# bramtoula/multi_robot_SLAM_separators

Hardware: AMD Instinct MI355X
Metric: candidate keyframe-pair verifications/sec (NetVLAD NN + ORB match + RANSAC) @1/2/4/8 GPU (higher is better)
Workload: dtype u8+f16+f32+f64

## Files before the change

### include/sepfinder.h

```cpp
#ifndef SEPFINDER_H
#define SEPFINDER_H

#include <stdint.h>
#include <stddef.h>

#ifdef __cplusplus
extern "C" {
#endif

#define SF_ABI_VERSION 8

enum {
  SF_OK = 0,
  SF_EINVAL = 1,
  SF_EHIP = 2,
  SF_ENOMEM = 3,
  SF_ERANGE = 4,
  SF_ENODEV = 5,
  SF_ERCCL = 6
};

#define SF_MAX_FEATURES   32767
#define SF_MAX_DESC_BYTES 64
#define SF_MAX_DESC_BYTES_F32 512
// ... 361 lines not shown
int  sf_prof_get(sf_handle h, int kernel, int64_t* launches, double* total_ms);
const char* sf_kernel_name(int kernel);

enum {
  SF_OPT_MATCH_MFMA = 0,
  SF_OPT_FUSED = 1,
  SF_OPT_OVERLAP = 2,
  SF_OPT_CHAIN_WAVES = 3,
  SF_OPT_NN_FULL_FILTER = 5,
  SF_OPT_STEP_OVERLAP = 6,
  SF_OPT_STEP_SPLIT = 7,
  SF_OPT_STEP_DEPTH = 8,
  SF_OPT_STEP_LANES = 9,
  SF_OPT_STEP_DEVICE_WALK = 10,
  SF_OPT_STEP_SPECULATE = 11,
  SF_OPT_DEBUG_CORR = 4
};
int  sf_set_option(sf_handle h, int32_t option, int32_t value);

#ifdef __cplusplus
}
#endif
#endif
```

### multi_robot_slam_separators_amd/_abi.py

```python
import ctypes as C

import numpy as np

SF_OK, SF_EINVAL, SF_EHIP, SF_ENOMEM, SF_ERANGE, SF_ENODEV, SF_ERCCL = range(7)
SF_MAX_FEATURES = 32767
SF_MAX_DESC_BYTES = 64
SF_MAX_DESC_BYTES_F32 = 512

(SF_K_MATCH, SF_K_RANSAC1, SF_K_GUIDED, SF_K_RANSAC2, SF_K_NN, SF_K_NN_SELECT, SF_K_NN_FILTER,
 SF_K_NN_REFINE, SF_K_FUSED, SF_K_NN_WALK, SF_K_BA, SF_K_GUIDED_TP, SF_K_COUNT) = range(13)
(SF_OPT_MATCH_MFMA, SF_OPT_FUSED, SF_OPT_OVERLAP, SF_OPT_CHAIN_WAVES, SF_OPT_DEBUG_CORR, SF_OPT_NN_FULL_FILTER,
 SF_OPT_STEP_OVERLAP, SF_OPT_STEP_SPLIT, SF_OPT_STEP_DEPTH, SF_OPT_STEP_LANES, SF_OPT_STEP_DEVICE_WALK,
 SF_OPT_STEP_SPECULATE) = range(12)

STATUS_NAMES = {0: "SF_OK", 1: "SF_EINVAL", 2: "SF_EHIP", 3: "SF_ENOMEM", 4: "SF_ERANGE", 5: "SF_ENODEV", 6: "SF_ERCCL"}


class Params(C.Structure):
    _fields_ = [
        ("netvlad_distance", C.c_double),
        ("netvlad_dimensions", C.c_int32),
        ("netvlad_max_matches_nb", C.c_int32),
        ("nn_precision", C.c_int32),
        ("min_inliers", C.c_int32),
        ("inlier_distance", C.c_float),
        ("iterations", C.c_int32),
        ("refine_iterations", C.c_int32),
        ("refine_sigma", C.c_double),
# ... 385 lines not shown
```

### multi_robot_slam_separators_amd/csrc/k_ransac.hip

```cpp
#include "sf_device_math.hpp"
#include "sf_internal.hpp"
#include "k_ba.hip"

namespace {

struct RansacLds {
  float4* src;
  float4* dst;
  float* d2;
  uint8_t* mask_a;
  uint8_t* mask_b;
  double* red;
  unsigned long long* sums;
  int* misc;
  float* hyp;
  int* hyp_cnt;
  float* best;
  float* bc;
  uint32_t* cidx;
};

__device__ __forceinline__ RansacLds ransac_carve(unsigned char* p, int kcap) {
  RansacLds L;
  L.src = (float4*)p; p += (size_t)kcap * 16;
  L.dst = (float4*)p; p += (size_t)kcap * 16;
  L.red = (double*)p; p += 64 * 8;
  L.sums = (unsigned long long*)p; p += 4 * 8;
  L.d2 = (float*)p; p += (size_t)kcap * 4;
  L.misc = (int*)p; p += 16 * 4;
  L.mask_a = p; p += kcap;
  L.mask_b = p; p += kcap;
  L.hyp = (float*)p; p += 12 * 64 * 4;
  L.hyp_cnt = (int*)p; p += 5 * 64 * 4;
  L.best = (float*)p; p += 16 * 4;
  L.bc = (float*)p; p += 16 * 4;
  L.cidx = (uint32_t*)p;
  return L;
}

__device__ __forceinline__ bool draw_sample(const RansacLds& L, uint64_t seed, uint32_t it, int max_checks,
                                            uint32_t m, double sdt, uint32_t& s0, uint32_t& s1, uint32_t& s2) {
  for (int a = 0; a < max_checks; ++a) {
    sfd::sample_triplet(seed, it, (uint32_t)a, m, s0, s1, s2);
    float4 p0 = L.src[s0], p1 = L.src[s1], p2 = L.src[s2];
    float ax = p1.x - p0.x, ay = p1.y - p0.y, az = p1.z - p0.z;
    float bx = p2.x - p0.x, by = p2.y - p0.y, bz = p2.z - p0.z;
// ... 273 lines not shown

__device__ __forceinline__ void write_null_pass(PassState& out, int matches) {
  PassState ps;
#pragma unroll
  for (int i = 0; i < 12; ++i) ps.T[i] = 0.f;
  ps.var = 1.0; ps.var_ang = 1.0;
  ps.is_null = 1;
  ps.inliers = 0;
  ps.matches = matches;
  ps.pad = 0;
  out = ps;
}

template <int DIR = 0, int NW = 4>
__device__ __forceinline__ void ransac_body(const StoreView& st, int pair, int sF, int sT, const uint32_t* cl, int n_corr,
                                            PassState& out, const DeviceParams& P, unsigned char* lds,
                                            int trace_base = 2, uint8_t* mask_out = nullptr) {
  constexpr int NT = 64 * NW;
  const int tid = (int)threadIdx.x;
  const int lane = tid & 63, wave = tid >> 6;
  const int kcap = st.kcap;
  const RansacLds L = ransac_carve(lds, kcap);

  const float* xF = st.xyz + (size_t)sF * kcap * 3;
  const float* xT = st.xyz + (size_t)sT * kcap * 3;
  if (tid < 16) L.misc[tid] = 0;
  __syncthreads();
  int m = 0;
  for (int base = 0; base < n_corr; base += NT) {
    const int i = base + tid;
    bool ok = false;
    float ax = 0, ay = 0, az = 0, bx = 0, by = 0, bz = 0;
    if (i < n_corr) {
      const uint32_t c = cl[i];
      const float* a = DIR ? xT + 3 * (c >> 16) : xF + 3 * (c & 0xFFFFu);
      const float* b = DIR ? xF + 3 * (c & 0xFFFFu) : xT + 3 * (c >> 16);
      ax = a[0]; ay = a[1]; az = a[2];
// ... 304 lines not shown
__device__ inline void pass_to3dof(PassState& ps, int times) {
  if (ps.is_null) return;
  for (int t = 0; t < times; ++t) sfd::to3dof_canon(ps.T);
}

template <int DIR>
__global__ void __launch_bounds__(SF_BLOCK, 4)
k_ransac(StoreView st, const int32_t* __restrict__ pair_from, const int32_t* __restrict__ pair_to,
         const int32_t* __restrict__ list, const int32_t* __restrict__ counter,
         const uint32_t* __restrict__ corr, const CorrHeader* __restrict__ hdr,
         PassState* __restrict__ pass, uint8_t* __restrict__ mask, int extra_3dof, DeviceParams P) {
  if ((int)blockIdx.x >= *counter) return;
  extern __shared__ __attribute__((aligned(16))) unsigned char smem_raw[];
  const int pair = list[blockIdx.x];
  ransac_body<DIR>(st, pair, pair_from[pair], pair_to[pair], corr + (size_t)pair * st.kcap, hdr[pair].n_corr,
                       pass[pair], P, smem_raw, 2, mask ? mask + (size_t)pair * st.kcap : nullptr);
  if (extra_3dof && threadIdx.x == 0) pass_to3dof(pass[pair], extra_3dof);
}

__global__ void __launch_bounds__(64)
k_merge_directions(const int32_t* __restrict__ list, const int32_t* __restrict__ counter, PassState* __restrict__ fwd,
                   const PassState* __restrict__ back, const uint8_t* __restrict__ mask_f,
                   const uint8_t* __restrict__ mask_b, int kcap, int extra_3dof) {
  if ((int)blockIdx.x >= *counter) return;
  const int pair = list[blockIdx.x], lane = threadIdx.x;
  int uni = 0;
  for (int i = lane; i < kcap; i += 64) uni += (mask_f[(size_t)pair * kcap + i] | mask_b[(size_t)pair * kcap + i]) ? 1 : 0;
  uni = sfd::wave_sum(uni);
  if (lane != 0) return;
  PassState a = fwd[pair];
  const PassState b = back[pair];
// ... 89 lines not shown
```

### multi_robot_slam_separators_amd/csrc/k_verify.hip

```cpp
#ifndef SF_PNP_CHAIN_OCC
#define SF_PNP_CHAIN_OCC 3
#endif
#ifndef SF_MATCH_PIPE
#define SF_MATCH_PIPE 1
#endif
#ifndef SF_PNP_CHAIN_OCC4
#define SF_PNP_CHAIN_OCC4 2
#endif
#include "k_match.hip"
#include "k_ransac.hip"
#include "k_guided.hip"
#include "k_pnp.hip"

namespace {

struct FusedTail {
  PassState pass1, pass2;
  CorrHeader hdr1, hdr2;
  uint8_t guided_flag;
  int32_t stream_slot;
};

struct BaHandover {
  uint8_t* mask1;
  uint8_t* mask2;
  uint8_t* est2;
};

__device__ __forceinline__ void stream_accepted(int pair, const sf_result* __restrict__ out, const DeviceParams& P,
                                                int32_t& s_slot) {
  const AcceptStream& S = P.accept;
  const int tid = (int)threadIdx.x;
  if (tid == 0) {
    const bool ok = out[pair].success != 0;
    if (S.flags) S.flags[pair] = ok ? 1 : 0;
    int slot = -1;
    if (ok) {
      const unsigned sl = atomicAdd(S.counter, 1u);
      if (sl < (unsigned)S.cap) { slot = (int)sl; S.index[sl] = pair; }
    }
    s_slot = slot;
  }
  __syncthreads();
// ... 6 lines not shown
}

template <int W, int NW = 4, int PART = 0>
__device__ __forceinline__ void chain_after_match(const StoreView& st, int pair, int sF, int sT, bool est1, FusedTail& T,
                                                  uint32_t* cl, unsigned char* chain_lds, uint32_t* __restrict__ corr2,
                                                  CorrHeader* __restrict__ hdr2, PassState* __restrict__ pass1,
                                                  PassState* __restrict__ pass2, uint8_t* __restrict__ guided_flag,
                                                  sf_result* __restrict__ out, const DeviceParams& P,
                                                  const BaHandover& H) {
  constexpr int NT = 64 * NW;
  const int tid = threadIdx.x;
  const int kcap = st.kcap;
  __builtin_amdgcn_s_setprio(3);
  if constexpr (PART != 2) {
    if (est1) {
      ransac_body<0, NW>(st, pair, sF, sT, cl, T.hdr1.n_corr, T.pass1, P, chain_lds, 2,
                         PART == 1 ? H.mask1 + (size_t)pair * kcap : nullptr);
      if constexpr (PART == 0) {
        if (P.force_3dof && tid == 0) pass_to3dof(T.pass1, 2);
      }
      __syncthreads();
    }
    if constexpr (PART == 1) {
      if (tid == 0) pass1[pair] = T.pass1;
      return;
    }
  }
  const bool est2 = guided_body<W, false, NW>(st, pair, sF, sT, T.pass1, T.pass2, T.guided_flag, cl, T.hdr2, nullptr, nullptr,
                                              P, reinterpret_cast<int*>(chain_lds));
  __syncthreads();
  if (P.dbg_corr || PART == 2) {
    const int n = T.hdr2.n_corr;
    for (int i = tid; i < n; i += NT) corr2[(size_t)pair * kcap + i] = cl[i];
    if (tid == 0) hdr2[pair] = T.hdr2;
  }
  if (est2) {
    ransac_body<0, NW>(st, pair, sF, sT, cl, T.hdr2.n_corr, T.pass2, P, chain_lds, 11,
                       PART == 2 ? H.mask2 + (size_t)pair * kcap : nullptr);
    if constexpr (PART == 0) {
      if (P.force_3dof && tid == 0) pass_to3dof(T.pass2, 1);
    }
    __syncthreads();
  }
  SF_TRACE_MARK(P, pair, 17);
  if constexpr (PART == 2) {
    if (tid == 0) { pass2[pair] = T.pass2; guided_flag[pair] = T.guided_flag; H.est2[pair] = est2 ? 1 : 0; }
    return;
  }
  if (tid == 0) {
    if (P.dbg_corr) { pass1[pair] = T.pass1; pass2[pair] = T.pass2; guided_flag[pair] = T.guided_flag; }
    finalize_one(T.pass1, T.pass2, T.guided_flag, out[pair]);
  }
  if (P.accept_on) stream_accepted(pair, out, P, T.stream_slot);
}
// ... 71 lines not shown
__global__ void __launch_bounds__(64 * NW, 4)
k_chain(StoreView st, const int32_t* __restrict__ pair_from, const int32_t* __restrict__ pair_to,
        const uint32_t* __restrict__ corr1, const CorrHeader* __restrict__ hdr1, PassState* __restrict__ pass1,
        uint32_t* __restrict__ corr2, CorrHeader* __restrict__ hdr2, PassState* __restrict__ pass2,
        uint8_t* __restrict__ guided_flag, const int32_t* __restrict__ list, const int32_t* __restrict__ counter,
        sf_result* __restrict__ out, DeviceParams P, int tail_off, BaHandover H) {
  extern __shared__ __attribute__((aligned(16))) unsigned char smem_raw[];
  if ((int)blockIdx.x >= *counter) return;
  const int pair = list[blockIdx.x];
  const int tid = threadIdx.x;
  const int kcap = st.kcap;
  const int sF = pair_from[pair], sT = pair_to[pair];
  FusedTail& T = *reinterpret_cast<FusedTail*>(smem_raw + tail_off);
  uint32_t* cl = reinterpret_cast<uint32_t*>(smem_raw);
  unsigned char* chain_lds = smem_raw + (size_t)kcap * 4;
  if constexpr (PART != 2) {
    const CorrHeader h1 = hdr1[pair];
    if (tid == 0) { T.hdr1 = h1; T.pass1 = pass1[pair]; }
    for (int i = tid; i < h1.n_corr; i += 64 * NW) cl[i] = corr1[(size_t)pair * kcap + i];
  } else {
    if (tid == 0) T.pass1 = pass1[pair];
  }
  __syncthreads();
  SF_TRACE_MARK(P, pair, 1);
  chain_after_match<W, NW, PART>(st, pair, sF, sT, true, T, cl, chain_lds, corr2, hdr2, pass1, pass2, guided_flag, out, P, H);
}

template <int W, int NQ, bool WIDE = false>
int launch_fused(sf_context* c, StoreView st, const int32_t* d_from, const int32_t* d_to, int n, sf_result* d_out,
                 size_t lds, int tail_off) {
  bool& attr_set = c->fused_attr[W == 16][NQ == 0][WIDE];
  if (lds > 64 * 1024 && !attr_set) {
    SF_HIP(c, hipFuncSetAttribute((const void*)k_verify_fused<W, NQ, WIDE>, hipFuncAttributeMaxDynamicSharedMemorySize,
                                  160 * 1024));
    attr_set = true;
  }
  hipLaunchKernelGGL((k_verify_fused<W, NQ, WIDE>), dim3(n), dim3(SF_BLOCK), lds, c->stream, st, d_from, d_to,
                     (uint32_t*)c->w->corr1.p, (CorrHeader*)c->w->hdr1.p, (PassState*)c->w->pass1.p, (uint32_t*)c->w->corr2.p,
                     (CorrHeader*)c->w->hdr2.p, (PassState*)c->w->pass2.p, (uint8_t*)c->w->flags.p, d_out, c->dparams,
                     tail_off, c->pair_src);
// ... 178 lines not shown
bool sf_split_pnp_applicable(const sf_context* c, const StoreView& st) {
  if (c->dparams.estimation_type != 1 || !c->fused || c->match_variant != 0 || c->params.desc_type != 0) return false;
  if (c->dparams.bidirectional) return false;
  if (!(c->match_mfma && st.kcap <= MF_MAX_ROWS)) return false;
  const int nc = c->dparams.grid_gx * c->dparams.grid_gy;
  const size_t lds = std::max((sf_pnp_lds_bytes(st.kcap, c->dparams.iterations) + 15) & ~(size_t)15,
                              sf_guided_lds_bytes(st.kcap, nc));
  return lds <= 160 * 1024 && sf_match_lds_bytes(st.kcap, st.w) <= 160 * 1024 &&
         (!c->dparams.bundle_adjustment || sf_ba_lds_bytes(st.kcap) <= 160 * 1024);
}

namespace {
template <int W, int NW, int PART>
int launch_chain(sf_context* c, StoreView st, const int32_t* d_from, const int32_t* d_to, int n, sf_result* d_out,
                 size_t lds, int tail_off, const BaHandover& H) {
  bool& attr_set = c->chain_attr[W == 16][PART][NW == 4 ? 2 : NW - 1];
  if (lds > 64 * 1024 && !attr_set) {
    SF_HIP(c, hipFuncSetAttribute((const void*)k_chain<W, NW, PART>, hipFuncAttributeMaxDynamicSharedMemorySize, 160 * 1024));
    attr_set = true;
  }
  int32_t* counters = (int32_t*)c->w->counters.p;
  hipLaunchKernelGGL((k_chain<W, NW, PART>), dim3(n), dim3(64 * NW), lds, c->stream, st, d_from, d_to,
                     (const uint32_t*)c->w->corr1.p, (const CorrHeader*)c->w->hdr1.p, (PassState*)c->w->pass1.p,
                     (uint32_t*)c->w->corr2.p, (CorrHeader*)c->w->hdr2.p, (PassState*)c->w->pass2.p, (uint8_t*)c->w->flags.p,
                     (const int32_t*)c->w->list1.p, (const int32_t*)(counters + 0), d_out, c->dparams, tail_off, H);
  return SF_OK;
}

template <int W, int PART, int NW>
int launch_chain_pnp(sf_context* c, StoreView st, const int32_t* d_from, const int32_t* d_to, int n, sf_result* d_out,
// ... 5 lines not shown
  if (lds > 64 * 1024 && !attr) {
    SF_HIP(c, hipFuncSetAttribute((const void*)k_chain_pnp<W, PART, NW>, hipFuncAttributeMaxDynamicSharedMemorySize, 160 * 1024));
    attr = true;
  }
  int32_t* counters = (int32_t*)c->w->counters.p;
  hipLaunchKernelGGL((k_chain_pnp<W, PART, NW>), dim3(n), dim3(64 * NW), lds, c->stream, st, d_from, d_to,
                     (const uint32_t*)c->w->corr1.p, (const CorrHeader*)c->w->hdr1.p, (PassState*)c->w->pass1.p,
                     (uint32_t*)c->w->corr2.p, (CorrHeader*)c->w->hdr2.p, (PassState*)c->w->pass2.p, (uint8_t*)c->w->flags.p,
                     (const int32_t*)c->w->list1.p, (const int32_t*)(counters + 0), d_out, c->dparams, H);
  return SF_OK;
}

template <int PART>
int launch_chain_part(sf_context* c, StoreView st, const int32_t* d_from, const int32_t* d_to, int n, sf_result* d_out,
                      bool pnp, const BaHandover& H) {
  int rc;
  sf_prof_begin(c, SF_K_FUSED);
  if (pnp) {
#define SF_CHAIN_PNP_CASE(W_)                                                                            \
    rc = c->chain_pnp_nw == 1   ? launch_chain_pnp<W_, PART, 1>(c, st, d_from, d_to, n, d_out, H)          \
         : c->chain_pnp_nw == 2 ? launch_chain_pnp<W_, PART, 2>(c, st, d_from, d_to, n, d_out, H)          \
                                : launch_chain_pnp<W_, PART, 4>(c, st, d_from, d_to, n, d_out, H)
    if (st.w == 8) SF_CHAIN_PNP_CASE(8); else SF_CHAIN_PNP_CASE(16);
#undef SF_CHAIN_PNP_CASE
  } else {
    const int tail_off = (int)fused_tail_offset(c, st, false);
    const size_t lds_c = (size_t)tail_off + ((sizeof(FusedTail) + 15) & ~(size_t)15);
#define SF_CHAIN_CASE(W_)                                                                                             \
    rc = c->chain_nw == 1   ? launch_chain<W_, 1, PART>(c, st, d_from, d_to, n, d_out, lds_c, tail_off, H)            \
         : c->chain_nw == 2 ? launch_chain<W_, 2, PART>(c, st, d_from, d_to, n, d_out, lds_c, tail_off, H)            \
                            : launch_chain<W_, 4, PART>(c, st, d_from, d_to, n, d_out, lds_c, tail_off, H)
    if (st.w == 8) SF_CHAIN_CASE(8); else SF_CHAIN_CASE(16);
#undef SF_CHAIN_CASE
  }
  sf_prof_end(c, SF_K_FUSED);
  if (rc != SF_OK) return rc;
  SF_HIP(c, hipGetLastError());
  return SF_OK;
}
}

int sf_launch_verify_split(sf_context* c, StoreView st, const int32_t* d_from, const int32_t* d_to, int n,
                           sf_result* d_out) {
  if (n <= 0) return SF_OK;
  const bool pnp = c->dparams.estimation_type == 1;
  if (!(pnp ? sf_split_pnp_applicable(c, st) : sf_split_applicable(c, st)))
    return sf_fail(c, SF_EINVAL, "split verification pipeline not applicable");
  SF_HIP(c, hipMemsetAsync(c->w->counters.p, 0, 64, c->stream));
  const size_t lds_m = sf_match_lds_bytes(st.kcap, st.w);
  int32_t* counters = (int32_t*)c->w->counters.p;
  sf_prof_begin(c, SF_K_MATCH);
  if (lds_m > 64 * 1024 && !c->split_match_attr[st.w == 16]) {
    if (st.w == 8)
      SF_HIP(c, hipFuncSetAttribute((const void*)k_match_split<8>, hipFuncAttributeMaxDynamicSharedMemorySize, 160 * 1024));
    else
      SF_HIP(c, hipFuncSetAttribute((const void*)k_match_split<16>, hipFuncAttributeMaxDynamicSharedMemorySize, 160 * 1024));
    c->split_match_attr[st.w == 16] = true;
  }
#define SF_SPLIT_MATCH(...)                                                                                        \
  hipLaunchKernelGGL((k_match_split<__VA_ARGS__>), dim3(n), dim3(SF_BLOCK), lds_m, c->stream, st, d_from, d_to,    \
                     (uint32_t*)c->w->corr1.p, (CorrHeader*)c->w->hdr1.p, (PassState*)c->w->pass1.p, (CorrHeader*)c->w->hdr2.p, \
                     (PassState*)c->w->pass2.p, (uint8_t*)c->w->flags.p, (int32_t*)c->w->list1.p, counters + 0, d_out, c->dparams, \
                     sf_est_mode(c))
  if (st.w == 8) SF_SPLIT_MATCH(8); else SF_SPLIT_MATCH(16);
#undef SF_SPLIT_MATCH
  sf_prof_end(c, SF_K_MATCH);
  SF_HIP(c, hipGetLastError());
  if (!c->dparams.bundle_adjustment)
    return launch_chain_part<0>(c, st, d_from, d_to, n, d_out, pnp, BaHandover{nullptr, nullptr, nullptr});
  int rc;
  const size_t mb = (size_t)n * st.kcap;
  if ((rc = sf_buf_reserve(c, c->w->dir_mask, 2 * mb + (size_t)n)) != SF_OK) return rc;
  uint8_t* m1 = (uint8_t*)c->w->dir_mask.p;
  const BaHandover H = {m1, m1 + mb, m1 + 2 * mb};
  SF_HIP(c, hipMemsetAsync(m1, 0, 2 * mb + (size_t)n, c->stream));
  if ((rc = launch_chain_part<1>(c, st, d_from, d_to, n, d_out, pnp, H)) != SF_OK) return rc;
  if ((rc = sf_launch_ba_pass(c, st, d_from, d_to, n, 1, 1, H.mask1, nullptr, false, d_out)) != SF_OK) return rc;
  if ((rc = launch_chain_part<2>(c, st, d_from, d_to, n, d_out, pnp, H)) != SF_OK) return rc;
  return sf_launch_ba_pass(c, st, d_from, d_to, n, 2, 1, H.mask2, H.est2, true, d_out);
}
```

### multi_robot_slam_separators_amd/csrc/sf_handle.hip

```cpp
#include <math.h>
#include <stdarg.h>

#include "sf_host.hpp"

static thread_local std::string g_create_error;

int sf_fail(sf_context* c, int code, const char* fmt, ...) {
  char buf[512];
  va_list ap;
  va_start(ap, fmt);
  vsnprintf(buf, sizeof(buf), fmt, ap);
  va_end(ap);
  if (c) c->err = buf; else g_create_error = buf;
  return code;
}

int sf_buf_reserve(sf_context* c, Buf& b, size_t bytes, bool keep) {
  if (bytes <= b.bytes) return SF_OK;
  size_t want = std::max(bytes, b.bytes + b.bytes / 2);
  void* p = nullptr;
  hipError_t e = hipMalloc(&p, want);
  if (e != hipSuccess) return sf_fail(c, SF_ENOMEM, "hipMalloc(%zu) -> %s", want, hipGetErrorString(e));
  if (b.p) {
    if (keep && b.bytes) {
// ... 178 lines not shown
}

void sf_env_knobs(sf_context* c) {
  if (const char* v = getenv("SF_MATCH_VARIANT")) c->match_variant = atoi(v);
  if (const char* v = getenv("SF_FUSED")) {
    c->fused = atoi(v) != 0;
    c->split = atoi(v) == 2;
  }
  if (const char* v = getenv("SF_STEP_SPLIT_MIN")) c->split_auto_min = std::max(1, atoi(v));
  if (const char* v = getenv("SF_STEP_SPLIT")) c->split_auto = atoi(v) != 0;
  if (const char* v = getenv("SF_CHAIN_PNP")) c->chain_pnp = atoi(v) != 0;
  if (const char* v = getenv("SF_BA_OCC")) c->ba_occ = atoi(v) == 1 ? 1 : atoi(v) == 2 ? 2 : 0;
  if (const char* v = getenv("SF_BA_NW")) { const int nw = atoi(v); c->ba_nw = (nw == 1 || nw == 2) ? nw : 4; }
  if (const char* v = getenv("SF_CHAIN_PNP_NW")) { const int nw = atoi(v); c->chain_pnp_nw = (nw == 1 || nw == 2) ? nw : 4; }
  if (const char* v = getenv("SF_CHAIN_NW")) { const int nw = atoi(v); c->chain_nw = (nw == 1 || nw == 2) ? nw : 4; }
  if (const char* v = getenv("SF_MATCH_MFMA")) c->match_mfma = atoi(v) != 0;
  if (const char* v = getenv("SF_DEBUG_CORR")) c->debug_corr = atoi(v) != 0;
  if (const char* v = getenv("SF_OVERLAP")) c->overlap = atoi(v) != 0;
  if (const char* v = getenv("SF_STEP_OVERLAP")) c->step_overlap = atoi(v) != 0;
  if (const char* v = getenv("SF_OVERLAP_MIN")) c->overlap_min_pairs = std::max(2, atoi(v));
  if (const char* v = getenv("SF_STEP_DEPTH")) c->step_depth = std::max(1, std::min(SF_STEP_MAX_DEPTH, atoi(v)));
  if (const char* v = getenv("SF_STEP_LANES")) c->step_lanes = std::max(1, std::min(SF_STEP_MAX_LANES, atoi(v)));
  if (const char* v = getenv("SF_STEP_SPECULATE")) c->step_speculate = atoi(v) != 0;
  if (const char* v = getenv("SF_STEP_DEVICE_WALK")) c->step_device_walk = atoi(v) != 0;
}

extern "C" int sf_create(const sf_params* p, int device, sf_handle* out) {
  if (!out) return SF_EINVAL;
  *out = nullptr;
  int ndev = 0;
// ... 157 lines not shown
  if (launches) *launches = c->prof_slots[kernel].launches;
  if (total_ms) *total_ms = c->prof_slots[kernel].total_ms;
  return SF_OK;
}

extern "C" int sf_set_option(sf_handle c, int32_t option, int32_t value) {
  if (!c) return SF_EINVAL;
  switch (option) {
    case SF_OPT_MATCH_MFMA: c->match_mfma = value != 0; return SF_OK;
    case SF_OPT_FUSED: c->fused = value != 0; return SF_OK;
    case SF_OPT_OVERLAP: c->overlap = value != 0; return SF_OK;
    case SF_OPT_CHAIN_WAVES: return SF_OK;
    case SF_OPT_DEBUG_CORR: c->debug_corr = value != 0; return SF_OK;
    case SF_OPT_NN_FULL_FILTER: c->nn_force_full = value != 0; c->nn_coef_level = -1; return SF_OK;
    case SF_OPT_STEP_SPLIT: c->split_auto = value != 0; return SF_OK;
    case SF_OPT_STEP_OVERLAP:
      if (c->step_inflight) return sf_fail(c, SF_EINVAL, "SF_OPT_STEP_OVERLAP cannot change while steps are in flight");
      c->step_overlap = value != 0;
      return SF_OK;
    case SF_OPT_STEP_DEPTH:
      if (c->step_inflight) return sf_fail(c, SF_EINVAL, "SF_OPT_STEP_DEPTH cannot change while steps are in flight");
      if (value < 1 || value > SF_STEP_MAX_DEPTH) return sf_fail(c, SF_ERANGE, "SF_OPT_STEP_DEPTH %d not in 1..%d", value, SF_STEP_MAX_DEPTH);
      c->step_depth = value;
      c->step_seq = 0;
      return SF_OK;
    case SF_OPT_STEP_LANES:
      if (c->step_inflight) return sf_fail(c, SF_EINVAL, "SF_OPT_STEP_LANES cannot change while steps are in flight");
      if (value < 1 || value > SF_STEP_MAX_LANES) return sf_fail(c, SF_ERANGE, "SF_OPT_STEP_LANES %d not in 1..%d", value, SF_STEP_MAX_LANES);
      c->step_lanes = value;
      return SF_OK;
// ... 12 lines not shown
```

### multi_robot_slam_separators_amd/csrc/sf_host.hpp

```cpp
#pragma once
#include <stdio.h>
#include <stdlib.h>
#include <string.h>

#include <algorithm>
#include <utility>

#include "sf_internal.hpp"

int sf_fill_device_params(sf_context* c);
void sf_env_knobs(sf_context* c);

int sf_validate_features(sf_context* c, const sf_features* f);
int sf_store_reserve(sf_context* c, Store& s, int slots_needed, int rows, int cols);
int sf_store_add_host_batch(sf_context* c, Store& st, const sf_features* const* feats, int n, int* first_slot);
void sf_ingest_pool_destroy(sf_context* c);

struct VerifyPlan {
  enum Form { STAGES = 0, FUSED = 1, SPLIT = 2, SPLIT_PNP = 3, HALVES = 4 } form = STAGES;
  bool lists = true;
  bool single = false;
  bool streams() const { return single && (form == FUSED || form == SPLIT || form == SPLIT_PNP); }
};
VerifyPlan sf_verify_plan(const sf_context* c, const StoreView& v, int n);
int sf_verify_device(sf_context* c, const Store& st, const int32_t* d_from, const int32_t* d_to, int n, sf_result* d_out,
                     const VerifyPlan* given = nullptr);
int sf_compact_launch(sf_context* c, const sf_result* d_results, int n, sf_result* d_accepted, uint8_t* d_flags,
                      int32_t* d_count, const int32_t* index = nullptr, sf_result* d_accepted2 = nullptr,
                      uint8_t* d_flags2 = nullptr, int32_t* d_count2 = nullptr, int cap2 = 0x7FFFFFFF);

enum SideStream { SF_STREAM_COPY, SF_STREAM_LANE, SF_STREAM_AUX };
int sf_side_stream(sf_context* c, SideStream role, int k, hipStream_t* out);
```

### multi_robot_slam_separators_amd/csrc/sf_internal.hpp

```cpp
#pragma once
#include <hip/hip_runtime.h>
#include <stdint.h>
#include <string>
#include <vector>

#include "../../include/sepfinder.h"
#include "../../include/sf_experimental.h"

#define SF_BLOCK 256
#define SF_MAX_KCAP 4096
#define SF_STEP_MAX_DEPTH 16
#define SF_STEP_MAX_LANES 4

struct StoreView {
  const uint32_t* desc;
  const float* xyz;
  const float4* kp;
  const int4* meta;
  int kcap;
  int w;
  int n_slots;
};

struct PassState {
  float T[12];
  double var;
// ... 210 lines not shown

  int match_variant = 0;
  bool ransac_attr_set = false;
  bool pnp_attr_set = false;
  bool fused_attr[2][2][2] = {};
  bool ransac_ba_attr_set = false, pnp_ba_attr_set = false, merge_ba_attr_set = false;
  bool debug_corr = false;
  bool fused = true;
  int cu_count = 0;
  bool gf_select_attr = false;
  bool nn_t256_attr = false;
  bool split = false;
  bool split_auto = true;
  int split_auto_min = 2048;
  bool in_overlapped_step = false;
  bool chain_attr[2][3][3] = {};
  int chain_nw = 4;
  bool split_match_attr[2] = {};
  bool chain_pnp_attr[2][3][3] = {};
  int chain_pnp_nw = 2;
  bool ba_pass_attr[2][3] = {};
  int ba_occ = 0;
  int ba_nw = 1;
  bool chain_pnp = true;
  bool match_mfma = true;
  void* nn_pinned = nullptr;
  size_t nn_pinned_bytes = 0;

  void* pairs_pinned = nullptr;
  size_t pairs_pinned_bytes = 0;
  hipEvent_t pairs_staged = nullptr;
  int32_t* count_pinned = nullptr;
// ... 200 lines not shown
  return SF_OK;
}

int sf_launch_match_global(sf_context* c, StoreView st, const int32_t* d_from, const int32_t* d_to, int n);
int sf_launch_ransac(sf_context* c, StoreView st, const int32_t* d_from, const int32_t* d_to, int n, int pass);
int sf_launch_pnp(sf_context* c, StoreView st, const int32_t* d_from, const int32_t* d_to, int n, int pass);
int sf_launch_guided(sf_context* c, StoreView st, const int32_t* d_from, const int32_t* d_to, int n);
int sf_launch_ba_pass(sf_context* c, StoreView st, const int32_t* d_from, const int32_t* d_to, int n, int pass, int list_sel,
                      const uint8_t* mask, const uint8_t* run, bool fin, sf_result* d_out);
int sf_launch_merge_directions_ba(sf_context* c, StoreView st, const int32_t* d_from, const int32_t* d_to, int n, int pass,
                                  bool pnp, const uint8_t* mask_f, const uint8_t* mask_b);
size_t sf_fused_lds_bytes(const sf_context* c, const StoreView& st);
bool sf_split_applicable(const sf_context* c, const StoreView& st);
bool sf_split_pnp_applicable(const sf_context* c, const StoreView& st);
int sf_launch_verify_split(sf_context* c, StoreView st, const int32_t* d_from, const int32_t* d_to, int n,
                           sf_result* d_out);
int sf_launch_verify_fused(sf_context* c, StoreView st, const int32_t* d_from, const int32_t* d_to, int n,
                           sf_result* d_out);
size_t sf_ransac_lds_bytes(int kcap, int iterations);
size_t sf_ba_lds_bytes(int kcap);
size_t sf_pnp_lds_bytes(int kcap, int iterations);
size_t sf_guided_lds_bytes(int kcap, int n_cells, bool narrow = false);
void sf_brief_default_pattern(int8_t* tests, int bytes);
void sf_orb_default_pattern(int8_t* tests);
int sf_sort_keys(sf_context* c, const unsigned long long* in, unsigned long long* out, size_t n, unsigned bit0, unsigned bit1,
                 bool descending);
int sf_sort_keys_segmented(sf_context* c, const unsigned long long* in, unsigned long long* out, unsigned n_total,
                           unsigned n_segments, const unsigned* d_begin, const unsigned* d_end, unsigned bit0, unsigned bit1,
                           bool descending);
int sf_sort_keys_segmented_desc(sf_context* c, const unsigned long long* in, unsigned long long* out, unsigned n_total,
                                unsigned n_segments, const unsigned* d_begin, const unsigned* d_end, unsigned bit0,
// ... 92 lines not shown
```

### multi_robot_slam_separators_amd/csrc/sf_verify_host.hip

```cpp
#include "sf_host.hpp"

struct WsBytes { size_t corr1, corr2, hdr1, hdr2, pass1, pass2, list1, list3, flags; };
static size_t WsBytes::* const WS_ROW[9] = {&WsBytes::corr1, &WsBytes::corr2, &WsBytes::hdr1, &WsBytes::hdr2, &WsBytes::pass1,
                                            &WsBytes::pass2, &WsBytes::list1, &WsBytes::list3, &WsBytes::flags};
static Buf Workspace::* const WS_BUF[9] = {&Workspace::corr1, &Workspace::corr2, &Workspace::hdr1, &Workspace::hdr2, &Workspace::pass1,
                                           &Workspace::pass2, &Workspace::list1, &Workspace::list3, &Workspace::flags};
static WsBytes ws_bytes(int n, int kcap, bool lists) {
  const size_t np = (size_t)n;
  WsBytes w;
  w.corr1 = w.corr2 = lists ? np * kcap * 4 : 0;
  w.hdr1 = w.hdr2 = np * sizeof(CorrHeader);
  w.pass1 = w.pass2 = np * sizeof(PassState);
  w.list1 = w.list3 = np * 4;
  w.flags = np;
  return w;
}

static int ws_reserve(sf_context* c, int n, int kcap, bool lists) {
  int rc;
  const size_t np = (size_t)n;
  const WsBytes w = ws_bytes(n, kcap, lists);
  for (int i = 0; i < 9; ++i)
    if ((rc = sf_buf_reserve(c, c->w->*WS_BUF[i], w.*WS_ROW[i])) != SF_OK) return rc;
#ifndef SF_CHAIN_TRACE
// ... 21 lines not shown
static bool sf_use_split(const sf_context* c, const StoreView& v, int n) {
  if (c->split) return sf_split_applicable(c, v);
  if (c->dparams.bundle_adjustment && c->dparams.estimation_type == 0 && c->fused) return sf_split_applicable(c, v);
  if (!c->split_auto || !c->in_overlapped_step) return false;
  if (c->dparams.estimation_type != 0 || v.w != 8 || n > 65536 || n < c->split_auto_min || !sf_split_applicable(c, v))
    return false;
  return sf_fused_lds_bytes(c, v) * 4 <= 160 * 1024;
}

VerifyPlan sf_verify_plan(const sf_context* c, const StoreView& v, int n) {
  VerifyPlan p;
  if (c->overlap && n >= c->overlap_min_pairs) { p.form = VerifyPlan::HALVES; p.lists = true; p.single = false; return p; }
  p.single = n <= SF_CHUNK;
  if (c->dparams.guess_match_to_projection) { p.form = VerifyPlan::STAGES; p.lists = true; return p; }
  if (c->chain_pnp && sf_split_pnp_applicable(c, v)) { p.form = VerifyPlan::SPLIT_PNP; p.lists = true; }
  else if (sf_use_split(c, v, n)) { p.form = VerifyPlan::SPLIT; p.lists = true; }
  else if (sf_fused_lds_bytes(c, v) != 0 && !c->dparams.bundle_adjustment) { p.form = VerifyPlan::FUSED; p.lists = c->debug_corr; }
  else { p.form = VerifyPlan::STAGES; p.lists = true; }
  return p;
}

static WsBytes form_writes(VerifyPlan::Form form, int m, int kcap, bool debug_corr, bool ba) {
  const size_t np = (size_t)m, list = np * (size_t)kcap * 4;
  WsBytes w = {};
  switch (form) {
    case VerifyPlan::FUSED:
      if (debug_corr) { w.corr1 = w.corr2 = list; w.hdr1 = w.hdr2 = np * sizeof(CorrHeader); w.pass1 = w.pass2 = np * sizeof(PassState); w.flags = np; }
      break;
    case VerifyPlan::SPLIT:
      w.corr1 = list; w.hdr1 = np * sizeof(CorrHeader); w.pass1 = np * sizeof(PassState); w.list1 = np * 4;
      if (debug_corr || ba) { w.corr2 = list; w.hdr2 = np * sizeof(CorrHeader); w.pass2 = np * sizeof(PassState); w.flags = np; }
      break;
    case VerifyPlan::SPLIT_PNP:
    case VerifyPlan::STAGES:
    case VerifyPlan::HALVES:
      w.corr1 = w.corr2 = list; w.hdr1 = w.hdr2 = np * sizeof(CorrHeader); w.pass1 = w.pass2 = np * sizeof(PassState);
      w.list1 = w.list3 = np * 4; w.flags = np;
      break;
  }
  return w;
}

extern "C" int sf_debug_plan_workspace(const sf_params* p, int32_t kcap, int32_t desc_words, int32_t n_pairs,
                                       int32_t in_overlapped_step, int32_t debug_corr, int64_t* out, int32_t n_out) {
  if (!p || !out || n_out < 22 || kcap <= 0 || (kcap & 63) || (desc_words != 8 && desc_words != 16 && desc_words != 64 && desc_words != 128) || n_pairs <= 0)
    return SF_EINVAL;
// ... 1 lines not shown
  if (!c) return SF_ENOMEM;
  c->params = *p;
  int rc = sf_fill_device_params(c);
  if (rc == SF_OK) {
    sf_env_knobs(c);
    c->in_overlapped_step = in_overlapped_step != 0;
    c->debug_corr = debug_corr != 0;
    StoreView v = {};
    v.kcap = kcap; v.w = desc_words; v.n_slots = 1;
    const VerifyPlan plan = sf_verify_plan(c, v, n_pairs);
    const int seq = plan.form == VerifyPlan::HALVES ? std::min((std::min(n_pairs, 2 * SF_CHUNK) + 1) / 2, SF_CHUNK)
                                                    : std::min(n_pairs, SF_CHUNK);
    const bool lists = plan.form == VerifyPlan::HALVES ? true : plan.lists;
    const WsBytes r = ws_bytes(seq, kcap, lists);
    const WsBytes w = form_writes(plan.form == VerifyPlan::HALVES ? VerifyPlan::STAGES : plan.form, seq, kcap, c->debug_corr,
                                  c->dparams.bundle_adjustment != 0);
    out[0] = (int64_t)plan.form; out[1] = plan.lists; out[2] = plan.single; out[3] = seq;
    for (int i = 0; i < 9; ++i) { out[4 + i] = (int64_t)(r.*WS_ROW[i]); out[13 + i] = (int64_t)(w.*WS_ROW[i]); }
  }
  delete c;
  return rc;
}

static int verify_sequence(sf_context* c, const StoreView& view, const int32_t* d_from, const int32_t* d_to, int m,
                           sf_result* d_out, const VerifyPlan& plan) {
  int rc;
  c->dparams.dbg_corr = c->debug_corr ? 1 : 0;
  switch (plan.form) {
    case VerifyPlan::SPLIT_PNP:
      c->w->last_lists_valid = true;
      return sf_launch_verify_split(c, view, d_from, d_to, m, d_out);
    case VerifyPlan::SPLIT:
      c->w->last_lists_valid = c->debug_corr || c->dparams.bundle_adjustment != 0;
      return sf_launch_verify_split(c, view, d_from, d_to, m, d_out);
    case VerifyPlan::FUSED:
      c->w->last_lists_valid = c->debug_corr;
      return sf_launch_verify_fused(c, view, d_from, d_to, m, d_out);
    default: break;
  }
  c->w->last_lists_valid = true;
  SF_HIP(c, hipMemsetAsync(c->w->counters.p, 0, 64, c->stream));
  if ((rc = sf_launch_match_global(c, view, d_from, d_to, m)) != SF_OK) return rc;
  const bool pnp = c->dparams.estimation_type == 1;
  if ((rc = (pnp ? sf_launch_pnp : sf_launch_ransac)(c, view, d_from, d_to, m, 1)) != SF_OK) return rc;
  if ((rc = sf_launch_guided(c, view, d_from, d_to, m)) != SF_OK) return rc;
  if ((rc = (pnp ? sf_launch_pnp : sf_launch_ransac)(c, view, d_from, d_to, m, 2)) != SF_OK) return rc;
  return sf_launch_finalize(c, m, d_out);
}

// ... 454 lines not shown
```

Baseline: 25.83 million.

## Run small-correspondence RANSAC passes in narrow one-wave kernels around the chain

```diff
diff --git a/include/sepfinder.h b/include/sepfinder.h
--- a/include/sepfinder.h
+++ b/include/sepfinder.h
@@ -399,6 +399,7 @@
   SF_OPT_STEP_LANES = 9,
   SF_OPT_STEP_DEVICE_WALK = 10,
   SF_OPT_STEP_SPECULATE = 11,
+  SF_OPT_CHAIN_NARROW_EST = 12,
   SF_OPT_DEBUG_CORR = 4
 };
 int  sf_set_option(sf_handle h, int32_t option, int32_t value);
diff --git a/multi_robot_slam_separators_amd/_abi.py b/multi_robot_slam_separators_amd/_abi.py
--- a/multi_robot_slam_separators_amd/_abi.py
+++ b/multi_robot_slam_separators_amd/_abi.py
@@ -11,7 +11,7 @@
  SF_K_NN_REFINE, SF_K_FUSED, SF_K_NN_WALK, SF_K_BA, SF_K_GUIDED_TP, SF_K_COUNT) = range(13)
 (SF_OPT_MATCH_MFMA, SF_OPT_FUSED, SF_OPT_OVERLAP, SF_OPT_CHAIN_WAVES, SF_OPT_DEBUG_CORR, SF_OPT_NN_FULL_FILTER,
  SF_OPT_STEP_OVERLAP, SF_OPT_STEP_SPLIT, SF_OPT_STEP_DEPTH, SF_OPT_STEP_LANES, SF_OPT_STEP_DEVICE_WALK,
- SF_OPT_STEP_SPECULATE) = range(12)
+ SF_OPT_STEP_SPECULATE, SF_OPT_CHAIN_NARROW_EST) = range(13)
 
 STATUS_NAMES = {0: "SF_OK", 1: "SF_EINVAL", 2: "SF_EHIP", 3: "SF_ENOMEM", 4: "SF_ERANGE", 5: "SF_ENODEV", 6: "SF_ERCCL"}
 
diff --git a/multi_robot_slam_separators_amd/csrc/k_ransac.hip b/multi_robot_slam_separators_amd/csrc/k_ransac.hip
--- a/multi_robot_slam_separators_amd/csrc/k_ransac.hip
+++ b/multi_robot_slam_separators_amd/csrc/k_ransac.hip
@@ -20,16 +20,16 @@
   uint32_t* cidx;
 };
 
-__device__ __forceinline__ RansacLds ransac_carve(unsigned char* p, int kcap) {
+__device__ __forceinline__ RansacLds ransac_carve(unsigned char* p, int mcap) {
   RansacLds L;
-  L.src = (float4*)p; p += (size_t)kcap * 16;
-  L.dst = (float4*)p; p += (size_t)kcap * 16;
+  L.src = (float4*)p; p += (size_t)mcap * 16;
+  L.dst = (float4*)p; p += (size_t)mcap * 16;
   L.red = (double*)p; p += 64 * 8;
   L.sums = (unsigned long long*)p; p += 4 * 8;
-  L.d2 = (float*)p; p += (size_t)kcap * 4;
+  L.d2 = (float*)p; p += (size_t)mcap * 4;
   L.misc = (int*)p; p += 16 * 4;
-  L.mask_a = p; p += kcap;
-  L.mask_b = p; p += kcap;
+  L.mask_a = p; p += mcap;
+  L.mask_b = p; p += mcap;
   L.hyp = (float*)p; p += 12 * 64 * 4;
   L.hyp_cnt = (int*)p; p += 5 * 64 * 4;
   L.best = (float*)p; p += 16 * 4;
@@ -333,13 +333,13 @@
 
 template <int DIR = 0, int NW = 4>
 __device__ __forceinline__ void ransac_body(const StoreView& st, int pair, int sF, int sT, const uint32_t* cl, int n_corr,
-                                            PassState& out, const DeviceParams& P, unsigned char* lds,
+                                            PassState& out, const DeviceParams& P, unsigned char* lds, int mcap,
                                             int trace_base = 2, uint8_t* mask_out = nullptr) {
   constexpr int NT = 64 * NW;
   const int tid = (int)threadIdx.x;
   const int lane = tid & 63, wave = tid >> 6;
   const int kcap = st.kcap;
-  const RansacLds L = ransac_carve(lds, kcap);
+  const RansacLds L = ransac_carve(lds, mcap);
 
   const float* xF = st.xyz + (size_t)sF * kcap * 3;
   const float* xT = st.xyz + (size_t)sT * kcap * 3;
@@ -674,7 +674,7 @@
   extern __shared__ __attribute__((aligned(16))) unsigned char smem_raw[];
   const int pair = list[blockIdx.x];
   ransac_body<DIR>(st, pair, pair_from[pair], pair_to[pair], corr + (size_t)pair * st.kcap, hdr[pair].n_corr,
-                       pass[pair], P, smem_raw, 2, mask ? mask + (size_t)pair * st.kcap : nullptr);
+                       pass[pair], P, smem_raw, st.kcap, 2, mask ? mask + (size_t)pair * st.kcap : nullptr);
   if (extra_3dof && threadIdx.x == 0) pass_to3dof(pass[pair], extra_3dof);
 }
 
diff --git a/multi_robot_slam_separators_amd/csrc/k_verify.hip b/multi_robot_slam_separators_amd/csrc/k_verify.hip
--- a/multi_robot_slam_separators_amd/csrc/k_verify.hip
+++ b/multi_robot_slam_separators_amd/csrc/k_verify.hip
@@ -27,6 +27,10 @@
   uint8_t* est2;
 };
 
+#ifndef SF_EST_CAP
+#define SF_EST_CAP 256
+#endif
+
 __device__ __forceinline__ void stream_accepted(int pair, const sf_result* __restrict__ out, const DeviceParams& P,
                                                 int32_t& s_slot) {
   const AcceptStream& S = P.accept;
@@ -63,9 +67,9 @@
   __builtin_amdgcn_s_setprio(3);
   if constexpr (PART != 2) {
     if (est1) {
-      ransac_body<0, NW>(st, pair, sF, sT, cl, T.hdr1.n_corr, T.pass1, P, chain_lds, 2,
+      ransac_body<0, NW>(st, pair, sF, sT, cl, T.hdr1.n_corr, T.pass1, P, chain_lds, kcap, 2,
                          PART == 1 ? H.mask1 + (size_t)pair * kcap : nullptr);
-      if constexpr (PART == 0) {
+      if constexpr (PART == 0 || PART == 3) {
         if (P.force_3dof && tid == 0) pass_to3dof(T.pass1, 2);
       }
       __syncthreads();
@@ -78,15 +82,24 @@
   const bool est2 = guided_body<W, false, NW>(st, pair, sF, sT, T.pass1, T.pass2, T.guided_flag, cl, T.hdr2, nullptr, nullptr,
                                               P, reinterpret_cast<int*>(chain_lds));
   __syncthreads();
-  if (P.dbg_corr || PART == 2) {
+  const bool hand_over = PART == 3 && !(est2 && T.hdr2.n_corr > SF_EST_CAP);
+  if (P.dbg_corr || PART == 2 || hand_over) {
     const int n = T.hdr2.n_corr;
     for (int i = tid; i < n; i += NT) corr2[(size_t)pair * kcap + i] = cl[i];
     if (tid == 0) hdr2[pair] = T.hdr2;
   }
+  if constexpr (PART == 3) {
+    if (tid == 0) {
+      if (est1) pass1[pair] = T.pass1;
+      H.est2[pair] = hand_over ? (est2 ? 1 : 0) : 2;
+      if (hand_over) { pass2[pair] = T.pass2; guided_flag[pair] = T.guided_flag; }
+    }
+    if (hand_over) return;
+  }
   if (est2) {
-    ransac_body<0, NW>(st, pair, sF, sT, cl, T.hdr2.n_corr, T.pass2, P, chain_lds, 11,
+    ransac_body<0, NW>(st, pair, sF, sT, cl, T.hdr2.n_corr, T.pass2, P, chain_lds, kcap, 11,
                        PART == 2 ? H.mask2 + (size_t)pair * kcap : nullptr);
-    if constexpr (PART == 0) {
+    if constexpr (PART == 0 || PART == 3) {
       if (P.force_3dof && tid == 0) pass_to3dof(T.pass2, 1);
     }
     __syncthreads();
@@ -188,16 +201,54 @@
   FusedTail& T = *reinterpret_cast<FusedTail*>(smem_raw + tail_off);
   uint32_t* cl = reinterpret_cast<uint32_t*>(smem_raw);
   unsigned char* chain_lds = smem_raw + (size_t)kcap * 4;
+  bool est1 = true;
   if constexpr (PART != 2) {
     const CorrHeader h1 = hdr1[pair];
+    if constexpr (PART == 3) est1 = h1.n_corr > SF_EST_CAP;
     if (tid == 0) { T.hdr1 = h1; T.pass1 = pass1[pair]; }
-    for (int i = tid; i < h1.n_corr; i += 64 * NW) cl[i] = corr1[(size_t)pair * kcap + i];
+    if (est1)
+      for (int i = tid; i < h1.n_corr; i += 64 * NW) cl[i] = corr1[(size_t)pair * kcap + i];
   } else {
     if (tid == 0) T.pass1 = pass1[pair];
   }
   __syncthreads();
-  SF_TRACE_MARK(P, pair, 1);
-  chain_after_match<W, NW, PART>(st, pair, sF, sT, true, T, cl, chain_lds, corr2, hdr2, pass1, pass2, guided_flag, out, P, H);
+  if (PART != 3 || est1) SF_TRACE_MARK(P, pair, 1);
+  chain_after_match<W, NW, PART>(st, pair, sF, sT, est1, T, cl, chain_lds, corr2, hdr2, pass1, pass2, guided_flag, out, P, H);
+}
+
+template <int PASS>
+__global__ void __launch_bounds__(64, 4)
+k_chain_est(StoreView st, const int32_t* __restrict__ pair_from, const int32_t* __restrict__ pair_to,
+            const uint32_t* __restrict__ corr, const CorrHeader* __restrict__ hdr, PassState* __restrict__ pass1,
+            PassState* __restrict__ pass2, const uint8_t* __restrict__ guided_flag, const uint8_t* __restrict__ est2,
+            const int32_t* __restrict__ list, const int32_t* __restrict__ counter, sf_result* __restrict__ out,
+            DeviceParams P) {
+  extern __shared__ __attribute__((aligned(16))) unsigned char smem_raw[];
+  if ((int)blockIdx.x >= *counter) return;
+  const int pair = list[blockIdx.x];
+  const int run = PASS == 1 ? 1 : est2[pair];
+  if (run == 2) return;
+  const int n_corr = hdr[pair].n_corr;
+  if (PASS == 1 && n_corr > SF_EST_CAP) return;
+  __builtin_amdgcn_s_setprio(3);
+  if constexpr (PASS == 1) {
+    SF_TRACE_MARK(P, pair, 1);
+    ransac_body<0, 1>(st, pair, pair_from[pair], pair_to[pair], corr + (size_t)pair * st.kcap, n_corr, pass1[pair], P,
+                      smem_raw, SF_EST_CAP, 2);
+    if (P.force_3dof && threadIdx.x == 0) pass_to3dof(pass1[pair], 2);
+  } else {
+    if (run) {
+      ransac_body<0, 1>(st, pair, pair_from[pair], pair_to[pair], corr + (size_t)pair * st.kcap, n_corr, pass2[pair], P,
+                        smem_raw, SF_EST_CAP, 11);
+      if (P.force_3dof && threadIdx.x == 0) pass_to3dof(pass2[pair], 1);
+    }
+    SF_TRACE_MARK(P, pair, 17);
+    if (threadIdx.x == 0) finalize_one(pass1[pair], pass2[pair], guided_flag[pair], out[pair]);
+    if (P.accept_on) {
+      __syncthreads();
+      stream_accepted(pair, out, P, *reinterpret_cast<int32_t*>(smem_raw));
+    }
+  }
 }
 
 template <int W, int NQ, bool WIDE = false>
@@ -406,6 +457,7 @@
 template <int W, int NW, int PART>
 int launch_chain(sf_context* c, StoreView st, const int32_t* d_from, const int32_t* d_to, int n, sf_result* d_out,
                  size_t lds, int tail_off, const BaHandover& H) {
+  static_assert(PART >= 0 && PART <= 3, "chain_attr has one row per part");
   bool& attr_set = c->chain_attr[W == 16][PART][NW == 4 ? 2 : NW - 1];
   if (lds > 64 * 1024 && !attr_set) {
     SF_HIP(c, hipFuncSetAttribute((const void*)k_chain<W, NW, PART>, hipFuncAttributeMaxDynamicSharedMemorySize, 160 * 1024));
@@ -441,15 +493,18 @@
 template <int PART>
 int launch_chain_part(sf_context* c, StoreView st, const int32_t* d_from, const int32_t* d_to, int n, sf_result* d_out,
                       bool pnp, const BaHandover& H) {
-  int rc;
-  sf_prof_begin(c, SF_K_FUSED);
+  int rc = SF_OK;
+  if (PART == 3 && pnp) return sf_fail(c, SF_EINVAL, "the PnP chain has no three-launch form");
+  if (PART != 3) sf_prof_begin(c, SF_K_FUSED);
   if (pnp) {
+   if constexpr (PART != 3) {
 #define SF_CHAIN_PNP_CASE(W_)                                                                            \
     rc = c->chain_pnp_nw == 1   ? launch_chain_pnp<W_, PART, 1>(c, st, d_from, d_to, n, d_out, H)          \
          : c->chain_pnp_nw == 2 ? launch_chain_pnp<W_, PART, 2>(c, st, d_from, d_to, n, d_out, H)          \
                                 : launch_chain_pnp<W_, PART, 4>(c, st, d_from, d_to, n, d_out, H)
     if (st.w == 8) SF_CHAIN_PNP_CASE(8); else SF_CHAIN_PNP_CASE(16);
 #undef SF_CHAIN_PNP_CASE
+   }
   } else {
     const int tail_off = (int)fused_tail_offset(c, st, false);
     const size_t lds_c = (size_t)tail_off + ((sizeof(FusedTail) + 15) & ~(size_t)15);
@@ -460,15 +515,30 @@
     if (st.w == 8) SF_CHAIN_CASE(8); else SF_CHAIN_CASE(16);
 #undef SF_CHAIN_CASE
   }
-  sf_prof_end(c, SF_K_FUSED);
+  if (PART != 3) sf_prof_end(c, SF_K_FUSED);
   if (rc != SF_OK) return rc;
   SF_HIP(c, hipGetLastError());
   return SF_OK;
 }
 }
 
+namespace {
+template <int PASS>
+int launch_chain_est(sf_context* c, StoreView st, const int32_t* d_from, const int32_t* d_to, int n, sf_result* d_out,
+                     const BaHandover& H) {
+  int32_t* counters = (int32_t*)c->w->counters.p;
+  hipLaunchKernelGGL((k_chain_est<PASS>), dim3(n), dim3(64), sf_ransac_lds_bytes_dev(SF_EST_CAP), c->stream, st, d_from, d_to,
+                     (const uint32_t*)(PASS == 1 ? c->w->corr1.p : c->w->corr2.p),
+                     (const CorrHeader*)(PASS == 1 ? c->w->hdr1.p : c->w->hdr2.p), (PassState*)c->w->pass1.p,
+                     (PassState*)c->w->pass2.p, (const uint8_t*)c->w->flags.p, (const uint8_t*)H.est2,
+                     (const int32_t*)c->w->list1.p, (const int32_t*)(counters + 0), d_out, c->dparams);
+  SF_HIP(c, hipGetLastError());
+  return SF_OK;
+}
+}
+
 int sf_launch_verify_split(sf_context* c, StoreView st, const int32_t* d_from, const int32_t* d_to, int n,
-                           sf_result* d_out) {
+                           sf_result* d_out, bool narrow_est) {
   if (n <= 0) return SF_OK;
   const bool pnp = c->dparams.estimation_type == 1;
   if (!(pnp ? sf_split_pnp_applicable(c, st) : sf_split_applicable(c, st)))
@@ -493,9 +563,20 @@
 #undef SF_SPLIT_MATCH
   sf_prof_end(c, SF_K_MATCH);
   SF_HIP(c, hipGetLastError());
+  int rc;
+  if (narrow_est) {
+    if (pnp || c->dparams.bundle_adjustment) return sf_fail(c, SF_EINVAL, "narrow estimates: 3D-3D without bundle adjustment only");
+    if ((rc = sf_buf_reserve(c, c->w->dir_mask, (size_t)n)) != SF_OK) return rc;
+    const BaHandover H = {nullptr, nullptr, (uint8_t*)c->w->dir_mask.p};
+    sf_prof_begin(c, SF_K_FUSED);
+    if ((rc = launch_chain_est<1>(c, st, d_from, d_to, n, d_out, H)) == SF_OK &&
+        (rc = launch_chain_part<3>(c, st, d_from, d_to, n, d_out, false, H)) == SF_OK)
+      rc = launch_chain_est<2>(c, st, d_from, d_to, n, d_out, H);
+    sf_prof_end(c, SF_K_FUSED);
+    return rc;
+  }
   if (!c->dparams.bundle_adjustment)
     return launch_chain_part<0>(c, st, d_from, d_to, n, d_out, pnp, BaHandover{nullptr, nullptr, nullptr});
-  int rc;
   const size_t mb = (size_t)n * st.kcap;
   if ((rc = sf_buf_reserve(c, c->w->dir_mask, 2 * mb + (size_t)n)) != SF_OK) return rc;
   uint8_t* m1 = (uint8_t*)c->w->dir_mask.p;
diff --git a/multi_robot_slam_separators_amd/csrc/sf_handle.hip b/multi_robot_slam_separators_amd/csrc/sf_handle.hip
--- a/multi_robot_slam_separators_amd/csrc/sf_handle.hip
+++ b/multi_robot_slam_separators_amd/csrc/sf_handle.hip
@@ -216,6 +216,7 @@
   if (const char* v = getenv("SF_BA_NW")) { const int nw = atoi(v); c->ba_nw = (nw == 1 || nw == 2) ? nw : 4; }
   if (const char* v = getenv("SF_CHAIN_PNP_NW")) { const int nw = atoi(v); c->chain_pnp_nw = (nw == 1 || nw == 2) ? nw : 4; }
   if (const char* v = getenv("SF_CHAIN_NW")) { const int nw = atoi(v); c->chain_nw = (nw == 1 || nw == 2) ? nw : 4; }
+  if (const char* v = getenv("SF_CHAIN_NARROW_EST")) c->chain_narrow_est = atoi(v) != 0;
   if (const char* v = getenv("SF_MATCH_MFMA")) c->match_mfma = atoi(v) != 0;
   if (const char* v = getenv("SF_DEBUG_CORR")) c->debug_corr = atoi(v) != 0;
   if (const char* v = getenv("SF_OVERLAP")) c->overlap = atoi(v) != 0;
@@ -403,6 +404,7 @@
     case SF_OPT_DEBUG_CORR: c->debug_corr = value != 0; return SF_OK;
     case SF_OPT_NN_FULL_FILTER: c->nn_force_full = value != 0; c->nn_coef_level = -1; return SF_OK;
     case SF_OPT_STEP_SPLIT: c->split_auto = value != 0; return SF_OK;
+    case SF_OPT_CHAIN_NARROW_EST: c->chain_narrow_est = value != 0; return SF_OK;
     case SF_OPT_STEP_OVERLAP:
       if (c->step_inflight) return sf_fail(c, SF_EINVAL, "SF_OPT_STEP_OVERLAP cannot change while steps are in flight");
       c->step_overlap = value != 0;
diff --git a/multi_robot_slam_separators_amd/csrc/sf_host.hpp b/multi_robot_slam_separators_amd/csrc/sf_host.hpp
--- a/multi_robot_slam_separators_amd/csrc/sf_host.hpp
+++ b/multi_robot_slam_separators_amd/csrc/sf_host.hpp
@@ -20,6 +20,7 @@
   enum Form { STAGES = 0, FUSED = 1, SPLIT = 2, SPLIT_PNP = 3, HALVES = 4 } form = STAGES;
   bool lists = true;
   bool single = false;
+  bool narrow_est = false;
   bool streams() const { return single && (form == FUSED || form == SPLIT || form == SPLIT_PNP); }
 };
 VerifyPlan sf_verify_plan(const sf_context* c, const StoreView& v, int n);
diff --git a/multi_robot_slam_separators_amd/csrc/sf_internal.hpp b/multi_robot_slam_separators_amd/csrc/sf_internal.hpp
--- a/multi_robot_slam_separators_amd/csrc/sf_internal.hpp
+++ b/multi_robot_slam_separators_amd/csrc/sf_internal.hpp
@@ -10,6 +10,7 @@
 #define SF_BLOCK 256
 #define SF_MAX_KCAP 4096
 #define SF_STEP_MAX_DEPTH 16
+#define SF_CHAIN_NARROW_EST_DEFAULT true
 #define SF_STEP_MAX_LANES 4
 
 struct StoreView {
@@ -250,8 +251,9 @@
   bool split_auto = true;
   int split_auto_min = 2048;
   bool in_overlapped_step = false;
-  bool chain_attr[2][3][3] = {};
+  bool chain_attr[2][4][3] = {};
   int chain_nw = 4;
+  bool chain_narrow_est = SF_CHAIN_NARROW_EST_DEFAULT;
   bool split_match_attr[2] = {};
   bool chain_pnp_attr[2][3][3] = {};
   int chain_pnp_nw = 2;
@@ -482,7 +484,7 @@
 bool sf_split_applicable(const sf_context* c, const StoreView& st);
 bool sf_split_pnp_applicable(const sf_context* c, const StoreView& st);
 int sf_launch_verify_split(sf_context* c, StoreView st, const int32_t* d_from, const int32_t* d_to, int n,
-                           sf_result* d_out);
+                           sf_result* d_out, bool narrow_est = false);
 int sf_launch_verify_fused(sf_context* c, StoreView st, const int32_t* d_from, const int32_t* d_to, int n,
                            sf_result* d_out);
 size_t sf_ransac_lds_bytes(int kcap, int iterations);
diff --git a/multi_robot_slam_separators_amd/csrc/sf_verify_host.hip b/multi_robot_slam_separators_amd/csrc/sf_verify_host.hip
--- a/multi_robot_slam_separators_amd/csrc/sf_verify_host.hip
+++ b/multi_robot_slam_separators_amd/csrc/sf_verify_host.hip
@@ -59,13 +59,16 @@
   p.single = n <= SF_CHUNK;
   if (c->dparams.guess_match_to_projection) { p.form = VerifyPlan::STAGES; p.lists = true; return p; }
   if (c->chain_pnp && sf_split_pnp_applicable(c, v)) { p.form = VerifyPlan::SPLIT_PNP; p.lists = true; }
-  else if (sf_use_split(c, v, n)) { p.form = VerifyPlan::SPLIT; p.lists = true; }
+  else if (sf_use_split(c, v, n)) {
+    p.form = VerifyPlan::SPLIT; p.lists = true;
+    p.narrow_est = c->chain_narrow_est && !c->dparams.bundle_adjustment && c->dparams.adaptive_stop != 0;
+  }
   else if (sf_fused_lds_bytes(c, v) != 0 && !c->dparams.bundle_adjustment) { p.form = VerifyPlan::FUSED; p.lists = c->debug_corr; }
   else { p.form = VerifyPlan::STAGES; p.lists = true; }
   return p;
 }
 
-static WsBytes form_writes(VerifyPlan::Form form, int m, int kcap, bool debug_corr, bool ba) {
+static WsBytes form_writes(VerifyPlan::Form form, int m, int kcap, bool debug_corr, bool ba, bool narrow_est) {
   const size_t np = (size_t)m, list = np * (size_t)kcap * 4;
   WsBytes w = {};
   switch (form) {
@@ -74,7 +77,7 @@
       break;
     case VerifyPlan::SPLIT:
       w.corr1 = list; w.hdr1 = np * sizeof(CorrHeader); w.pass1 = np * sizeof(PassState); w.list1 = np * 4;
-      if (debug_corr || ba) { w.corr2 = list; w.hdr2 = np * sizeof(CorrHeader); w.pass2 = np * sizeof(PassState); w.flags = np; }
+      if (debug_corr || ba || narrow_est) { w.corr2 = list; w.hdr2 = np * sizeof(CorrHeader); w.pass2 = np * sizeof(PassState); w.flags = np; }
       break;
     case VerifyPlan::SPLIT_PNP:
     case VerifyPlan::STAGES:
@@ -106,7 +109,8 @@
     const bool lists = plan.form == VerifyPlan::HALVES ? true : plan.lists;
     const WsBytes r = ws_bytes(seq, kcap, lists);
     const WsBytes w = form_writes(plan.form == VerifyPlan::HALVES ? VerifyPlan::STAGES : plan.form, seq, kcap, c->debug_corr,
-                                  c->dparams.bundle_adjustment != 0);
+                                  c->dparams.bundle_adjustment != 0, plan.narrow_est);
+    if (n_out >= 23) out[22] = plan.narrow_est;
     out[0] = (int64_t)plan.form; out[1] = plan.lists; out[2] = plan.single; out[3] = seq;
     for (int i = 0; i < 9; ++i) { out[4 + i] = (int64_t)(r.*WS_ROW[i]); out[13 + i] = (int64_t)(w.*WS_ROW[i]); }
   }
@@ -124,7 +128,7 @@
       return sf_launch_verify_split(c, view, d_from, d_to, m, d_out);
     case VerifyPlan::SPLIT:
       c->w->last_lists_valid = c->debug_corr || c->dparams.bundle_adjustment != 0;
-      return sf_launch_verify_split(c, view, d_from, d_to, m, d_out);
+      return sf_launch_verify_split(c, view, d_from, d_to, m, d_out, plan.narrow_est);
     case VerifyPlan::FUSED:
       c->w->last_lists_valid = c->debug_corr;
       return sf_launch_verify_fused(c, view, d_from, d_to, m, d_out);
```

After: 26.27 million, median of 6. 1.7% higher.
